# google-research/multinerf

Hardware: NVIDIA H100
Metric: train-step rays/sec @16384 rays x (64+64+32) samples (higher is better)
Workload: dtype bf16

## Files before the change

include/mnrf.h:

```cpp
#ifndef MNRF_H_
#define MNRF_H_

#include <stddef.h>
#include <stdint.h>

#ifdef __cplusplus
extern "C" {
#endif

typedef uint16_t mnrf_bf16;
typedef void* mnrf_stream;

#define MNRF_ABI_VERSION 1

int mnrf_abi_version(void);
const char* mnrf_last_error(void);
int mnrf_device_ok(void);
int mnrf_num_sms(void);

typedef struct {
  int32_t num_rays, num_prev, num_samples;
  int32_t use_dilation;
  float dilation, domain_lo, domain_hi;
  float anneal, resample_padding;
  int32_t jitter_mode;
  float max_jitter;
} mnrf_sample_desc;

int mnrf_sample_level(const mnrf_sample_desc* d, const float* sdist_prev, const float* w_prev,
                      const float* u_base, const float* jitter, const float* cw_in,
                      float* sdist_out, int32_t* idx_out, float* cw_out, float* tdil_out,
                      float* wdil_out, mnrf_stream stream);
int mnrf_sample_level_dyn(const mnrf_sample_desc* d, const float* sdist_prev, const float* w_prev,
                          const float* u_base, const float* jitter, const float* anneal_dev,
                          float* sdist_out, mnrf_stream stream);

enum { MNRF_RAYDIST_NONE = 0, MNRF_RAYDIST_RECIPROCAL, MNRF_RAYDIST_LOG, MNRF_RAYDIST_EXP,
       MNRF_RAYDIST_SQRT, MNRF_RAYDIST_SQUARE, MNRF_RAYDIST_PIECEWISE };
enum { MNRF_RAY_CONE = 0, MNRF_RAY_CYLINDER = 1 };

typedef struct {
  int32_t num_rays, num_samples;
  int32_t raydist_fn, ray_shape, warp_contract, disable_integration;
  int32_t basis_k, min_deg, max_deg;
  int32_t ld_feat, feat_cols;
} mnrf_encode_desc;

int mnrf_encode(const mnrf_encode_desc* d, const float* sdist, const float* origins,
                const float* directions, const float* radii, const float* near,
                const float* far, const float* basis, mnrf_bf16* feat_bf16, float* feat_f32,
                float* tdist_out, mnrf_stream stream);
int mnrf_encode_tangent(const mnrf_encode_desc* d, const float* sdist, const float* origins,
                        const float* directions, const float* radii, const float* near,
                        const float* far, const float* basis, mnrf_bf16* feat_bf16,
                        mnrf_bf16* tfeat_bf16, int32_t ld_tfeat, mnrf_stream stream);

int mnrf_viewdir_enc(int32_t num_rays, int32_t num_samples, int32_t deg, const float* viewdirs,
                     mnrf_bf16* out, int32_t ld, int32_t col0, int32_t col_end,
                     mnrf_stream stream);

enum { MNRF_GEMM_FWD = 0, MNRF_GEMM_DGRAD = 1, MNRF_GEMM_WGRAD = 2 };
enum { MNRF_ACT_NONE = 0, MNRF_ACT_RELU = 1, MNRF_ACT_SOFTPLUS = 2, MNRF_ACT_SILU = 3 };

typedef struct {
  int32_t mode, act;
  int64_t m;
  int32_t n, k;
  int64_t lda, ldb, ldc, ldmask;
  int64_t ldmaskbits;
  int64_t ldadd;
  int64_t mask_mod;
  int32_t impl;
} mnrf_gemm_desc;

int mnrf_gemm(const mnrf_gemm_desc* d, const mnrf_bf16* a, const mnrf_bf16* b, const float* bias,
              const float* rowv, const float* colv, const mnrf_bf16* mask, uint32_t* maskbits,
              float* colsum, const mnrf_bf16* addend, void* out, mnrf_stream stream);

int mnrf_gemm_act(const mnrf_gemm_desc* d, const mnrf_bf16* a, const mnrf_bf16* b, const float* bias,
                  const float* rowv, const float* colv, float* colsum, const mnrf_bf16* addend, mnrf_bf16* z,
                  int64_t ldz, void* out, mnrf_stream stream);

int mnrf_gemm_wgrad(const mnrf_gemm_desc* d, const mnrf_bf16* a, const mnrf_bf16* b, float* bsum,
                    const float* side_w, float* side_aw, float* out, mnrf_stream stream);

typedef struct {
  int32_t block_n;
  int32_t staged;
  int32_t mask_tma;
  int32_t smooth;
  int32_t side;
  int32_t splits;
  int32_t tiles;
  int32_t grid;
} mnrf_gemm_instance;
int mnrf_gemm_plan(const mnrf_gemm_desc* d, const mnrf_bf16* a, const mnrf_bf16* b, const float* bias,
                   const float* rowv, const float* colv, const mnrf_bf16* mask, const uint32_t* maskbits,
                   const float* colsum, const mnrf_bf16* addend, const mnrf_bf16* z, int64_t ldz, const void* out,
                   const float* bsum, const float* side_w, const float* side_aw, mnrf_gemm_instance* plan);

#define MNRF_CHAIN_MAX_LAYERS 8
enum { MNRF_CHAIN_FWD = 0, MNRF_CHAIN_BWD = 1 };

typedef struct {
  const mnrf_bf16* w;
  int64_t ldw;
  const float* bias;
  uint32_t* maskbits;
  int64_t ldmaskbits;
  float* colsum;
  mnrf_bf16* out;
  int64_t ldo;
  int32_t n_stream, stream_col0, stream_kb0;
  int32_t n_res, res_kb0;
  int32_t reserved;
} mnrf_chain_layer;

typedef struct {
  int32_t mode, num_layers;
  int32_t width;
  int32_t stream_cols;
  int64_t m;
  const mnrf_bf16* stream;
  int64_t ldstream;
  const float* head_w;
  const float* head_b;
  float* head_out;
  int32_t head_n;
  int32_t reserved;
  mnrf_chain_layer layer[MNRF_CHAIN_MAX_LAYERS];
} mnrf_chain_desc;

int mnrf_mlp_chain(const mnrf_chain_desc* d, mnrf_stream stream);
int mnrf_mlp_chain_max_layers(void);

int mnrf_head_fwd(int64_t m, int32_t k, int32_t n_out, const mnrf_bf16* x, int64_t ldx,
                  const mnrf_bf16* w, const float* b, float* raw, mnrf_stream stream);
int mnrf_head_bwd(int64_t m, int32_t k, int32_t n_out, const mnrf_bf16* x, int64_t ldx,
                  const mnrf_bf16* w, const float* draw, mnrf_bf16* dx, int64_t lddx,
                  int32_t relu_mask, float* dw, float* dw2, int32_t dw_split, float* db, float* dxsum,
                  int32_t dx_cols, mnrf_bf16* dx2, int64_t lddx2, mnrf_stream stream);
int mnrf_head_bwd_act(int64_t m, int32_t k, int32_t n_out, const mnrf_bf16* x, int64_t ldx,
                      const mnrf_bf16* w, const float* draw, mnrf_bf16* dx, int64_t lddx,
                      int32_t act, const mnrf_bf16* z, int64_t ldz, float* dw, float* dw2, int32_t dw_split,
                      float* db, float* dxsum, int32_t dx_cols, mnrf_bf16* dx2, int64_t lddx2, mnrf_stream stream);

int mnrf_colsum(int64_t m, int32_t n, const mnrf_bf16* x, int64_t ldx, float* out,
                mnrf_stream stream);

enum { MNRF_RGB_SIGMOID = 0, MNRF_RGB_SAFE_EXP = 1 };

typedef struct {
  int32_t num_rays, num_samples;
  int32_t raydist_fn, opaque_background;
  float density_bias, density_noise;
  int32_t rgb_act;
  float rgb_premult, rgb_bias, rgb_padding;
  float bg_const;
  int32_t rgb_mode;
  int32_t ld_density, ld_rgb;
} mnrf_composite_desc;

int mnrf_composite_fwd(const mnrf_composite_desc* d, const float* raw_density,
                       const float* raw_rgb, const float* density_noise, const float* sdist,
                       const float* directions, const float* near, const float* far,
                       const float* bg_rgb, const float* rgb_scale, const float* raw_diffuse,
                       const float* raw_tint, float* weights, float* rgb_out,
                       float* density_out, float* rgb_samples, float* acc, float* dist,
                       mnrf_stream stream);

enum { MNRF_LOSS_MSE = 0, MNRF_LOSS_CHARB = 1, MNRF_LOSS_RAWNERF = 2 };

typedef struct {
  mnrf_composite_desc c;
  int32_t loss_type;
  float charb_padding;
  float data_mult;
  float distortion_mult;
  float interlevel_mult;
  int32_t num_samples_fine;
  int32_t lossmult_channels;
} mnrf_loss_desc;

int mnrf_composite_bwd(const mnrf_loss_desc* d, const float* raw_density, const float* raw_rgb,
                       const float* density_noise, const float* sdist, const float* directions,
                       const float* near, const float* far, const float* bg_rgb,
                       const float* rgb_scale, const float* raw_diffuse, const float* raw_tint,
                       const float* extra_dw ,
                       const float* target_rgb,
                       const float* lossmult, const float* inv_denom ,
                       const float* sdist_fine, const float* weights_fine,
                       float* d_raw_density, float* d_raw_rgb, float* d_rgb_scale ,
                       float* d_raw_diffuse, float* d_raw_tint, float* stats, mnrf_stream stream);
int mnrf_composite_bwd_masked(const mnrf_loss_desc* d, const float* raw_density, const float* raw_rgb,
                              const float* density_noise, const float* sdist, const float* directions,
                              const float* near, const float* far, const float* bg_rgb,
                              const float* rgb_scale, const float* raw_diffuse, const float* raw_tint,
                              const float* extra_dw, const float* target_rgb,
                              const float* lossmult, const float* inv_denom,
                              const float* sdist_fine, const float* weights_fine, const float* data_mask,
                              float* d_raw_density, float* d_raw_rgb, float* d_rgb_scale,
                              float* d_raw_diffuse, float* d_raw_tint, float* stats, mnrf_stream stream);
int mnrf_composite_bwd_chunk(const mnrf_loss_desc* d, const float* raw_density, const float* raw_rgb,
                             const float* density_noise, const float* sdist, const float* directions,
                             const float* near, const float* far, const float* bg_rgb,
                             const float* rgb_scale, const float* raw_diffuse, const float* raw_tint,
                             const float* extra_dw, const float* target_rgb,
                             const float* lossmult, const float* inv_denom,
                             const float* sdist_fine, const float* weights_fine, const float* data_mask,
                             float* d_raw_density, float* d_raw_rgb, float* d_rgb_scale,
                             float* d_raw_diffuse, float* d_raw_tint, float* stats, int32_t batch_rays,
                             mnrf_stream stream);

typedef struct {
  int32_t num_rays;
  int32_t patch_size, inner_patch_size, filter_size;
  int32_t enable;
  float smoothed_thresh;
  float patch_thresh;
} mnrf_robust_desc;

int mnrf_robust_mask(const mnrf_robust_desc* d, const float* rgb, const float* target, const float* threshold,
                     float* mask, float* error_per_pixel, uint32_t* counts, float* stats, mnrf_stream stream);
int mnrf_robust_mask_chunk(const mnrf_robust_desc* d, const float* rgb, const float* target, const float* threshold,
                           float* mask, float* error_per_pixel, uint32_t* counts, float* stats, int32_t batch_rays,
                           mnrf_stream stream);
int mnrf_quantile(int32_t n, float q, const float* x, float* out, mnrf_stream stream);

typedef struct {
  int64_t M;
  int32_t num_samples;
  int32_t use_pred_normals, use_density_normals, use_reflections, use_ide, use_n_dot_v, use_roughness;
  int32_t deg_view, ide_n;
  float roughness_bias;
  int32_t ld, col0, col_end;
} mnrf_refdir_desc;

int mnrf_refdir_fwd(const mnrf_refdir_desc* d, const float* ide_mat, const int32_t* ide_ml,
                    const float* grad_pred, const float* raw_rough, const float* raw_grad_density,
                    const float* viewdirs, float* normals_pred, float* normals, float* roughness,
                    mnrf_bf16* slab, float orient_mult, float prednorm_mult, int32_t orient_on_pred,
                    float* extra_dw , mnrf_stream stream);
int mnrf_refdir_bwd(const mnrf_refdir_desc* d, const float* ide_mat, const int32_t* ide_ml,
                    const float* grad_pred, const float* raw_rough, const float* raw_grad_density,
                    const float* viewdirs, const float* weights, mnrf_bf16* d_slab,
                    int32_t ld_dslab, float orient_mult, float prednorm_mult, int32_t orient_on_pred,
                    const float* d_raw_density, const float* d_raw_diffuse, const float* d_raw_tint,
// ... 79 lines not shown
```

multinerf_b200/csrc/gemm_tc.cu:

```cuda
#include <cuda.h>

#include <stdlib.h>
#include <string.h>

#include <algorithm>

#include "tc_common.cuh"

namespace mnrf {

constexpr int BLOCK_M = 128;
constexpr int BLOCK_K = 64;
constexpr int A_STAGE_BYTES = BLOCK_M * BLOCK_K * 2;
constexpr int NUM_THREADS = 384;
constexpr int CS_MAX = 1024;
constexpr int gemm_stages(int bn) { return bn == 256 ? 4 : bn == 128 ? 6 : 8; }
constexpr int STAGING_BLOCK_BYTES = 64 * 128;
constexpr int staging_blocks(int mode, int bn, bool ts) {
  return !ts ? 0 : (mode == MNRF_GEMM_FWD && bn >= 128) ? 2 : 1;
}
constexpr int mask_words(int bn) { return bn >= 128 ? bn / 32 : 0; }
constexpr int MASK_BUFS = 2;
constexpr int dgrad_smem_bytes(int bn) { return 8 * bn * 4 + MASK_BUFS * BLOCK_M * mask_words(bn) * 4; }
constexpr int SIDE_SCRATCH = 96 * 8;
// ... 265 lines not shown
      const bool leader = (threadIdx.x & 127) == 0;
      const uint32_t c_row = smem_u32(smem_c) + c * (SB * STAGING_BLOCK_BYTES) + (r_in - 64 * c) * 128 + (cq << 1);
      int64_t rows[2];
      bool row_ok[2];
      float rv[2] = {0.f, 0.f};
      const uint32_t* mrow[2] = {nullptr, nullptr};
#pragma unroll
      for (int h = 0; h < 2; ++h) {
        rows[h] = (int64_t)m_blk * BLOCK_M + r_in + 8 * h;
        row_ok[h] = rows[h] < p.m;
        if (MODE == MNRF_GEMM_DGRAD && row_ok[h]) {
          if (p.rowv) rv[h] = p.rowv[rows[h]];
          if (p.maskbits && !mask_tma)
            mrow[h] = p.maskbits + (p.mask_mod > 0 ? rows[h] % p.mask_mod : rows[h]) * p.ldmaskbits;
        }
      }
      const uint32_t m_row = smem_u32(mask_s) + ((it % MASK_BUFS) * BLOCK_M + r_in) * (MW * 4);
      if (mask_tma) mbar_wait(&mask_full[it % MASK_BUFS], (it / MASK_BUFS) & 1, 5);
      uint32_t bits[2] = {0u, 0u};
      uint32_t mw[2] = {0u, 0u};
#pragma unroll
      for (int i = 0; i < BN / 8; ++i) {
        const int col = ncol0 + 8 * i + cq;
        if (TS && SB == 1 && (i & 7) == 0) {
          if (leader) tma_store_wait_read<0>();
          named_bar_sync(2 + c, 128);
        }
        if (MODE == MNRF_GEMM_DGRAD && p.maskbits && (i & 3) == 0) {
#pragma unroll
          for (int h = 0; h < 2; ++h)
            mw[h] = mask_tma ? ld_shared_u32(m_row + (8 * h * MW + (i >> 2)) * 4)
                             : row_ok[h] ? __ldg(mrow[h] + (col >> 5)) : 0u;
        }
        float v[2][2];
#pragma unroll
        for (int h = 0; h < 2; ++h) { v[h][0] = acc[4 * i + 2 * h]; v[h][1] = acc[4 * i + 2 * h + 1]; }
        if (MODE == MNRF_GEMM_FWD) {
          if (p.bias) {
            const float2 b = __ldg(reinterpret_cast<const float2*>(p.bias + col));
#pragma unroll
            for (int h = 0; h < 2; ++h) { v[h][0] += b.x; v[h][1] += b.y; }
          }
          if constexpr (SMOOTH) {
#pragma unroll
            for (int h = 0; h < 2; ++h) {
              if (p.mask && row_ok[h])
                *reinterpret_cast<uint32_t*>(const_cast<__nv_bfloat16*>(p.mask) + rows[h] * p.ldmask + col) =
                    pack_bf16(v[h][0], v[h][1]);
              v[h][0] = act_fwd(p.act, v[h][0]);
              v[h][1] = act_fwd(p.act, v[h][1]);
            }
          } else if (p.act == MNRF_ACT_RELU) {
#pragma unroll
            for (int h = 0; h < 2; ++h)
#pragma unroll
              for (int e = 0; e < 2; ++e) {
                v[h][e] = fmaxf(v[h][e], 0.f);
                bits[h] |= (v[h][e] > 0.f ? 1u : 0u) << ((8 * i + cq + e) & 31);
              }
          }
        } else {
          float2 cv = make_float2(0.f, 0.f);
          if (p.rowv) cv = __ldg(reinterpret_cast<const float2*>(p.colv + col));
#pragma unroll
          for (int h = 0; h < 2; ++h) {
            if (p.rowv) { v[h][0] += rv[h] * cv.x; v[h][1] += rv[h] * cv.y; }
            if constexpr (SMOOTH) {
              if (row_ok[h]) {
                const int64_t zr = p.mask_mod > 0 ? rows[h] % p.mask_mod : rows[h];
                const uint32_t zz = __ldg(reinterpret_cast<const unsigned int*>(p.mask + zr * p.ldmask + col));
                v[h][0] *= act_d1(p.act, bf16_lo(zz));
                v[h][1] *= act_d1(p.act, bf16_hi(zz));
              }
            } else if (p.maskbits) {
              if (!((mw[h] >> (col & 31)) & 1u)) v[h][0] = 0.f;
              if (!((mw[h] >> ((col + 1) & 31)) & 1u)) v[h][1] = 0.f;
            } else if (p.mask && row_ok[h]) {
              const uint32_t mm = __ldg(reinterpret_cast<const unsigned int*>(p.mask + rows[h] * p.ldmask + col));
              if (!(bf16_lo(mm) > 0.f)) v[h][0] = 0.f;
              if (!(bf16_hi(mm) > 0.f)) v[h][1] = 0.f;
            }
            if (p.addend && row_ok[h]) {
              const uint32_t aa = __ldg(reinterpret_cast<const unsigned int*>(p.addend + rows[h] * p.ldadd + col));
              v[h][0] += bf16_lo(aa);
              v[h][1] += bf16_hi(aa);
            }
          }
          if (do_cs) {
            const bool hi = (lane >> 2) & 1;
            const float s0 = v[0][0] + v[1][0], s1 = v[0][1] + v[1][1];
            float t = (hi ? s1 : s0) + __shfl_xor_sync(0xffffffffu, hi ? s0 : s1, 4);
            t += __shfl_xor_sync(0xffffffffu, t, 8);
            t += __shfl_xor_sync(0xffffffffu, t, 16);
            if (lane < 8) {
              const uint32_t a = cs_lane + 8 * i * 4;
              st_shared_u32(a, __float_as_uint(__uint_as_float(ld_shared_u32(a)) + t));
            }
          }
        }
#pragma unroll
        for (int h = 0; h < 2; ++h) {
          if (TS) {
            st_shared_u32(c_row + ((i >> 3) & (SB - 1)) * STAGING_BLOCK_BYTES + h * (8 * 128) +
                              (((i & 7) ^ ((lane >> 2) & 7)) << 4),
                          pack_bf16(v[h][0], v[h][1]));
          } else if (row_ok[h]) {
            *reinterpret_cast<uint32_t*>(reinterpret_cast<__nv_bfloat16*>(p.out) + rows[h] * p.ldc + col) =
                pack_bf16(v[h][0], v[h][1]);
          }
        }
        if (MODE == MNRF_GEMM_FWD && p.act == MNRF_ACT_RELU && p.maskbits && (i & 3) == 3) {
#pragma unroll
          for (int h = 0; h < 2; ++h) {
            bits[h] |= __shfl_xor_sync(0xffffffffu, bits[h], 1);
            bits[h] |= __shfl_xor_sync(0xffffffffu, bits[h], 2);
            if ((lane & 3) == ((i >> 2) & 3) && row_ok[h]) p.maskbits[rows[h] * p.ldmaskbits + (col >> 5)] = bits[h];
            bits[h] = 0u;
          }
        }
        if (TS && (i & 7) == 7) {
          fence_proxy_async();
          if (SB == 2 && leader) tma_store_wait_read<0>();
          named_bar_sync(2 + c, 128);
          if (leader) {
            tma_store_2d(&tmap_c, smem_c + (c * SB + ((i >> 3) & (SB - 1))) * STAGING_BLOCK_BYTES, ncol0 + 8 * (i & ~7),
                         (int)((int64_t)m_blk * BLOCK_M + 64 * c));
            tma_store_commit();
          }
        }
      }
      if (mask_tma) {
        __syncwarp();
        if (lane == 0) mbar_arrive(&mask_empty[it % MASK_BUFS]);
      }
      const int next = tile + (int)gridDim.x;
      if (do_cs && (next >= total_tiles || next % p.num_n_blocks != n_blk)) {
        named_bar_sync(1, 2 * 128);
        for (int j = threadIdx.x - 128; j < BN; j += 2 * 128) {
          float s = 0.f;
#pragma unroll
          for (int sw = 0; sw < 8; ++sw) {
            s += cs_s[sw * BN + j];
            cs_s[sw * BN + j] = 0.f;
          }
          atomicAdd(p.colsum + ncol0 + j, s);
        }
        named_bar_sync(1, 2 * 128);
      }
    }
    if (TS && (threadIdx.x & 127) == 0) tma_store_wait_all();
  }
}

template <int MODE, int BN, bool TS, bool SIDE, bool SMOOTH>
static int launch_gemm_tc(int grid, const CUtensorMap& ta, const CUtensorMap& tb, const CUtensorMap& tc,
                          const CUtensorMap& tm, const GemmParams& p, cudaStream_t stream) {
  static bool attr_set = false;
  constexpr int kSmem = smem_bytes(MODE, BN, TS, SIDE);
  static_assert(kSmem <= 232448, "shared memory budget");
  auto kern = gemm_tc_kernel<MODE, BN, TS, SIDE, SMOOTH>;
  if (!attr_set) {
    MNRF_CUDA(cudaFuncSetAttribute(kern, cudaFuncAttributeMaxDynamicSharedMemorySize, kSmem));
    attr_set = true;
  }
  cudaLaunchConfig_t cfg = {};
  cfg.gridDim = dim3(grid); cfg.blockDim = dim3(NUM_THREADS);
  cfg.dynamicSmemBytes = kSmem; cfg.stream = stream;
  cudaLaunchAttribute attr[1];
  attr[0].id = cudaLaunchAttributeProgrammaticStreamSerialization;
  attr[0].val.programmaticStreamSerializationAllowed = 1;
  cfg.attrs = attr; cfg.numAttrs = pdl_enabled() ? 1 : 0;
  MNRF_CUDA(cudaLaunchKernelEx(&cfg, kern, ta, tb, tc, tm, p));
  return 0;
}

int gemm_tc_smooth_launch(int mode, int block_n, int grid, const CUtensorMap& ta, const CUtensorMap& tb,
                          const CUtensorMap& tc, const GemmParams& p, cudaStream_t stream);

#ifndef MNRF_GEMM_TC_SMOOTH_UNIT
static int pick_block_n(int n) {
  const int cands[] = {256, 128, 64, 32, 16};
  for (int c : cands)
    if (n % c == 0) return c;
  return 0;
}

static int gemm_tc_plan(const mnrf_gemm_desc* d, const mnrf_bf16* a, const mnrf_bf16* b, const float* bias,
                        const float* colv, const mnrf_bf16* mask, const uint32_t* maskbits, const float* colsum,
                        const mnrf_bf16* addend, const void* out, const float* bsum, const float* side_w,
                        const float* side_aw, const mnrf_bf16* z, int64_t ldz, mnrf_gemm_instance* plan) {
  MNRF_CHECK(d->mode == MNRF_GEMM_WGRAD || d->k % BLOCK_K == 0,
             "mnrf_gemm(tc): reduction length %d must be a multiple of %d", d->k, BLOCK_K);
  MNRF_CHECK(d->lda % 8 == 0 && d->ldb % 8 == 0 && ((uintptr_t)a % 16) == 0 && ((uintptr_t)b % 16) == 0,
             "mnrf_gemm(tc): operands must be 16-byte aligned with ld %% 8 == 0");
  const int block_n = pick_block_n(d->n);
  MNRF_CHECK(block_n > 0, "mnrf_gemm(tc): N=%d must be a multiple of 16", d->n);
  if (d->mode == MNRF_GEMM_WGRAD)
    MNRF_CHECK(block_n >= 64, "mnrf_gemm(tc): WGRAD needs N %% 64 == 0 (MN-major 128-byte atoms), N=%d", d->n);
  if (addend) MNRF_CHECK(d->mode == MNRF_GEMM_DGRAD && d->ldadd % 2 == 0 && ((uintptr_t)addend % 4) == 0,
                         "mnrf_gemm(tc): addend is a DGRAD input with 4-byte aligned rows");
  if (colsum) MNRF_CHECK(d->mode == MNRF_GEMM_DGRAD && d->n <= CS_MAX,
                         "mnrf_gemm(tc): colsum is a DGRAD output of at most %d columns", CS_MAX);
  const bool side = bsum != nullptr || side_aw != nullptr;
  if (side) MNRF_CHECK(d->mode == MNRF_GEMM_WGRAD && (side_w == nullptr) == (side_aw == nullptr),
                       "mnrf_gemm(tc): side sums are WGRAD outputs; side_w and side_aw come together");
  if (maskbits) {
    MNRF_CHECK(d->mode != MNRF_GEMM_WGRAD, "mnrf_gemm(tc): maskbits make no sense for WGRAD");
    MNRF_CHECK(d->n % 32 == 0 && block_n % 32 == 0 && d->ldmaskbits * 32 >= d->n,
               "mnrf_gemm(tc): maskbits need N %% 32 == 0 and ldmaskbits >= N/32");
  }
  const bool smooth = d->mode != MNRF_GEMM_WGRAD && (d->act == MNRF_ACT_SOFTPLUS || d->act == MNRF_ACT_SILU);
  if (smooth) {
    MNRF_CHECK(!maskbits && !mask, "mnrf_gemm(tc): a smooth activation takes z, not a ReLU mask");
    MNRF_CHECK(d->mode == MNRF_GEMM_FWD || z, "mnrf_gemm(tc): the DGRAD of a smooth activation needs z");
    MNRF_CHECK(!z || (ldz % 2 == 0 && ((uintptr_t)z % 4) == 0), "mnrf_gemm(tc): z must be 4-byte aligned");
  }
  if (bias) MNRF_CHECK(((uintptr_t)bias % 8) == 0, "mnrf_gemm(tc): bias must be 8-byte aligned");
  if (colv) MNRF_CHECK(((uintptr_t)colv % 8) == 0, "mnrf_gemm(tc): colv must be 8-byte aligned");
  const int workers = mnrf_num_sms();
  const int num_m_blocks = (int)((d->m + BLOCK_M - 1) / BLOCK_M);
  const int num_n_blocks = d->n / block_n;
  const int num_k_blocks = (d->k + BLOCK_K - 1) / BLOCK_K;
  int num_splits = 1;
  if (d->mode == MNRF_GEMM_WGRAD) {
    const int out_tiles = num_m_blocks * num_n_blocks;
    const int max_splits = std::min(std::max(1, (2 * workers) / out_tiles), num_k_blocks);
    int splits = max_splits;
    for (int sp = 1; sp <= max_splits; ++sp) {
      const int items = out_tiles * sp;
      const int rounds = (items + workers - 1) / workers;
      if (items * 100 >= rounds * workers * 95) { splits = sp; break; }
    }
    num_splits = splits;
  }
  const int kblocks_per_split = (num_k_blocks + num_splits - 1) / num_splits;
  num_splits = (num_k_blocks + kblocks_per_split - 1) / kblocks_per_split;
  if (d->mode != MNRF_GEMM_WGRAD) {
    MNRF_CHECK(d->ldc % 2 == 0 && ((uintptr_t)out % 4) == 0, "mnrf_gemm(tc): bf16 output must be 4-byte aligned");
    if (mask) MNRF_CHECK(d->ldmask % 2 == 0 && ((uintptr_t)mask % 4) == 0, "mnrf_gemm(tc): mask must be 4-byte aligned");
  } else {
    MNRF_CHECK(d->ldc % 2 == 0 && ((uintptr_t)out % 8) == 0, "mnrf_gemm(tc): fp32 output must be 8-byte aligned");
  }
  const bool ts = d->mode != MNRF_GEMM_WGRAD && block_n >= 64 && ((uintptr_t)out % 16) == 0 && d->ldc % 8 == 0;
  MNRF_CHECK(!smooth || ts, "mnrf_gemm(tc): a smooth activation needs N %% 64 == 0 and a 16-byte aligned output "
             "with a row pitch that is a multiple of 8");
  const bool mask_tma = d->mode == MNRF_GEMM_DGRAD && maskbits && mask_words(block_n) > 0 && d->ldmaskbits % 4 == 0 &&
                        ((uintptr_t)maskbits % 16) == 0 && (d->mask_mod == 0 || d->mask_mod % BLOCK_M == 0);
  const int tiles = num_m_blocks * num_n_blocks * num_splits;
  plan->block_n = block_n;
  plan->staged = ts;
  plan->mask_tma = mask_tma;
  plan->smooth = smooth;
  plan->side = side;
  plan->splits = num_splits;
  plan->tiles = tiles;
  plan->grid = std::min(tiles, workers);
  return 0;
}

int gemm_tc_launch(const mnrf_gemm_desc* d, const mnrf_bf16* a, const mnrf_bf16* b, const float* bias,
                   const float* rowv, const float* colv, const mnrf_bf16* mask, uint32_t* maskbits,
                   float* colsum, const mnrf_bf16* addend, void* out, cudaStream_t stream, float* bsum,
                   const float* side_w, float* side_aw, mnrf_bf16* z, int64_t ldz) {
  mnrf_gemm_instance plan;
  if (int rc = gemm_tc_plan(d, a, b, bias, colv, mask, maskbits, colsum, addend, out, bsum, side_w, side_aw, z, ldz,
                            &plan))
    return rc;
  const int block_n = plan.block_n;
  const bool ts = plan.staged, side = plan.side, smooth = plan.smooth;
  GemmParams p{};
  p.mode = d->mode; p.act = d->act; p.m = d->m; p.n = d->n; p.k = d->k;
  p.num_m_blocks = (int)((d->m + BLOCK_M - 1) / BLOCK_M);
  p.num_n_blocks = d->n / block_n;
  p.num_k_blocks = (d->k + BLOCK_K - 1) / BLOCK_K;
  p.num_splits = plan.splits;
  p.kblocks_per_split = (p.num_k_blocks + p.num_splits - 1) / p.num_splits;
  p.ldc = d->ldc; p.ldmask = d->ldmask;
  p.bias = bias; p.rowv = rowv; p.colv = colv;
  p.mask = reinterpret_cast<const __nv_bfloat16*>(mask);
  p.out = out;
  p.maskbits = maskbits;
  p.ldmaskbits = d->ldmaskbits;
  p.mask_mod = d->mask_mod;
  p.addend = reinterpret_cast<const __nv_bfloat16*>(addend);
  p.ldadd = d->ldadd;
  p.colsum = colsum;
  p.bsum = bsum; p.side_w = side_w; p.side_aw = side_aw;
  if (smooth) {
    p.mask = reinterpret_cast<const __nv_bfloat16*>(z);
    p.ldmask = ldz;
  }
  p.mask_tma = plan.mask_tma;
  CUtensorMap ta, tb, tc;
  if (d->mode != MNRF_GEMM_WGRAD) {
    if (make_tmap(&ta, a, d->m, d->k, d->lda, BLOCK_K, BLOCK_M)) return 1;
    if (make_tmap(&tb, b, d->n, d->k, d->ldb, BLOCK_K, block_n)) return 1;
  } else {
    if (make_tmap(&ta, a, d->k, d->m, d->lda, 64, BLOCK_K)) return 1;
    if (make_tmap(&tb, b, d->k, d->n, d->ldb, 64, BLOCK_K)) return 1;
  }
  if (ts) {
    if (make_tmap(&tc, out, d->m, d->n, d->ldc, 64, 64)) return 1;
  } else {
    tc = tb;
  }
  CUtensorMap tm = tb;
  if (p.mask_tma &&
      make_tmap(&tm, maskbits, d->mask_mod > 0 ? d->mask_mod : d->m, d->n / 32, d->ldmaskbits,
                mask_words(block_n), BLOCK_M, CU_TENSOR_MAP_DATA_TYPE_UINT32, 4,
                CU_TENSOR_MAP_SWIZZLE_NONE))
    return 1;
  const int grid = plan.grid;
  if (grid == 0) return 0;
#define MNRF_LAUNCH_TC3(MODE_, BN_, TS_, SIDE_)                                                       \
  do {                                                                                                \
    if (int rc = launch_gemm_tc<MODE_, BN_, TS_, SIDE_, false>(grid, ta, tb, tc, tm, p, stream)) return rc; \
  } while (0)
#define MNRF_LAUNCH_TC2(MODE_, BN_)                                                                   \
  do {                                                                                                \
    if (side) MNRF_LAUNCH_TC3(MODE_, BN_, false, MODE_ == MNRF_GEMM_WGRAD && BN_ >= 64);              \
    else if (ts) MNRF_LAUNCH_TC3(MODE_, BN_, MODE_ != MNRF_GEMM_WGRAD && BN_ >= 64, false);           \
    else MNRF_LAUNCH_TC3(MODE_, BN_, false, false);                                                   \
  } while (0)
#define MNRF_LAUNCH_TC(MODE_)                                                                         \
  do {                                                                                                \
    switch (block_n) {                                                                                \
      case 256: MNRF_LAUNCH_TC2(MODE_, 256); break;                                                   \
      case 128: MNRF_LAUNCH_TC2(MODE_, 128); break;                                                   \
      case 64: MNRF_LAUNCH_TC2(MODE_, 64); break;                                                     \
      case 32: if (MODE_ != MNRF_GEMM_WGRAD) MNRF_LAUNCH_TC2(MODE_, 32); break;                       \
      default: if (MODE_ != MNRF_GEMM_WGRAD) MNRF_LAUNCH_TC2(MODE_, 16); break;                       \
    }                                                                                                 \
  } while (0)
  if (smooth) {
    if (int rc = gemm_tc_smooth_launch(d->mode, block_n, grid, ta, tb, tc, p, stream)) return rc;
  } else if (d->mode == MNRF_GEMM_FWD) MNRF_LAUNCH_TC(MNRF_GEMM_FWD);
  else if (d->mode == MNRF_GEMM_DGRAD) MNRF_LAUNCH_TC(MNRF_GEMM_DGRAD);
  else MNRF_LAUNCH_TC(MNRF_GEMM_WGRAD);
  MNRF_LAUNCH_CHECK();
  return 0;
}
#endif

}

#ifndef MNRF_GEMM_TC_SMOOTH_UNIT
extern "C" int mnrf_gemm_plan(const mnrf_gemm_desc* d, const mnrf_bf16* a, const mnrf_bf16* b, const float* bias,
                              const float* rowv, const float* colv, const mnrf_bf16* mask, const uint32_t* maskbits,
                              const float* colsum, const mnrf_bf16* addend, const mnrf_bf16* z, int64_t ldz,
                              const void* out, const float* bsum, const float* side_w, const float* side_aw,
                              mnrf_gemm_instance* plan) {
  MNRF_CHECK(d && plan, "mnrf_gemm_plan: null pointer");
  MNRF_CHECK((rowv == nullptr) == (colv == nullptr), "mnrf_gemm: rowv and colv come together");
  MNRF_CHECK(!mask || d->mask_mod == 0, "mnrf_gemm: mask_mod applies to maskbits and z, not to a bf16 mask");
  return mnrf::gemm_tc_plan(d, a, b, bias, colv, mask, maskbits, colsum, addend, out, bsum, side_w, side_aw, z, ldz,
                            plan);
}
#endif
```

multinerf_b200/lib.py:

```python
import ctypes as C
import os

import torch

_HERE = os.path.dirname(os.path.abspath(__file__))
LIB_PATH = os.environ.get('MNRF_LIB') or os.path.join(_HERE, 'libmnrf_b200.so')


class MnrfError(RuntimeError):
  pass


class SampleDesc(C.Structure):
  _fields_ = [('num_rays', C.c_int32), ('num_prev', C.c_int32), ('num_samples', C.c_int32),
              ('use_dilation', C.c_int32), ('dilation', C.c_float), ('domain_lo', C.c_float),
              ('domain_hi', C.c_float), ('anneal', C.c_float), ('resample_padding', C.c_float),
              ('jitter_mode', C.c_int32), ('max_jitter', C.c_float)]


class EncodeDesc(C.Structure):
  _fields_ = [('num_rays', C.c_int32), ('num_samples', C.c_int32), ('raydist_fn', C.c_int32),
              ('ray_shape', C.c_int32), ('warp_contract', C.c_int32),
              ('disable_integration', C.c_int32), ('basis_k', C.c_int32), ('min_deg', C.c_int32),
              ('max_deg', C.c_int32), ('ld_feat', C.c_int32), ('feat_cols', C.c_int32)]


class GemmDesc(C.Structure):
  _fields_ = [('mode', C.c_int32), ('act', C.c_int32), ('m', C.c_int64), ('n', C.c_int32),
              ('k', C.c_int32), ('lda', C.c_int64), ('ldb', C.c_int64), ('ldc', C.c_int64),
              ('ldmask', C.c_int64), ('ldmaskbits', C.c_int64), ('ldadd', C.c_int64),
              ('mask_mod', C.c_int64),
              ('impl', C.c_int32)]


class GemmInstance(C.Structure):
  _fields_ = [('block_n', C.c_int32), ('staged', C.c_int32), ('mask_tma', C.c_int32), ('smooth', C.c_int32),
              ('side', C.c_int32), ('splits', C.c_int32), ('tiles', C.c_int32), ('grid', C.c_int32)]


class CompositeDesc(C.Structure):
  _fields_ = [('num_rays', C.c_int32), ('num_samples', C.c_int32), ('raydist_fn', C.c_int32),
              ('opaque_background', C.c_int32), ('density_bias', C.c_float),
              ('density_noise', C.c_float), ('rgb_act', C.c_int32), ('rgb_premult', C.c_float),
              ('rgb_bias', C.c_float), ('rgb_padding', C.c_float), ('bg_const', C.c_float),
              ('rgb_mode', C.c_int32), ('ld_density', C.c_int32), ('ld_rgb', C.c_int32)]


class LossDesc(C.Structure):
  _fields_ = [('c', CompositeDesc), ('loss_type', C.c_int32), ('charb_padding', C.c_float),
              ('data_mult', C.c_float), ('distortion_mult', C.c_float),
              ('interlevel_mult', C.c_float), ('num_samples_fine', C.c_int32),
              ('lossmult_channels', C.c_int32)]


class RobustDesc(C.Structure):
  _fields_ = [('num_rays', C.c_int32), ('patch_size', C.c_int32), ('inner_patch_size', C.c_int32),
              ('filter_size', C.c_int32), ('enable', C.c_int32), ('smoothed_thresh', C.c_float),
              ('patch_thresh', C.c_float)]


class RefdirDesc(C.Structure):
  _fields_ = [('M', C.c_int64), ('num_samples', C.c_int32), ('use_pred_normals', C.c_int32),
              ('use_density_normals', C.c_int32), ('use_reflections', C.c_int32), ('use_ide', C.c_int32),
              ('use_n_dot_v', C.c_int32), ('use_roughness', C.c_int32), ('deg_view', C.c_int32),
              ('ide_n', C.c_int32), ('roughness_bias', C.c_float), ('ld', C.c_int32), ('col0', C.c_int32),
              ('col_end', C.c_int32)]


class CameraDesc(C.Structure):
  _fields_ = [('num_rays', C.c_int32), ('num_cameras', C.c_int32), ('camtype', C.c_int32),
              ('has_distortion', C.c_int32), ('k1', C.c_float), ('k2', C.c_float), ('k3', C.c_float),
              ('k4', C.c_float), ('p1', C.c_float), ('p2', C.c_float), ('undistort_eps', C.c_float),
              ('undistort_iters', C.c_int32), ('has_ndc', C.c_int32), ('ndc_p02', C.c_float),
              ('ndc_p12', C.c_float), ('ndc_near', C.c_float)]


class SphericalDesc(C.Structure):
  _fields_ = [('height', C.c_int32), ('width', C.c_int32), ('camtoworld', C.c_double * 12)]


class PackItem(C.Structure):
  _fields_ = [('master', C.c_void_p), ('w_nk', C.c_void_p), ('w_kn', C.c_void_p), ('in_pad', C.c_int32),
              ('out', C.c_int32), ('tile0', C.c_int32), ('reserved', C.c_int32)]


CHAIN_MAX_LAYERS = 8
CHAIN_FWD, CHAIN_BWD = 0, 1


class ChainLayer(C.Structure):
  _fields_ = [('w', C.c_void_p), ('ldw', C.c_int64), ('bias', C.c_void_p), ('maskbits', C.c_void_p),
              ('ldmaskbits', C.c_int64), ('colsum', C.c_void_p), ('out', C.c_void_p), ('ldo', C.c_int64),
              ('n_stream', C.c_int32), ('stream_col0', C.c_int32), ('stream_kb0', C.c_int32),
              ('n_res', C.c_int32), ('res_kb0', C.c_int32), ('reserved', C.c_int32)]


class ChainDesc(C.Structure):
  _fields_ = [('mode', C.c_int32), ('num_layers', C.c_int32), ('width', C.c_int32), ('stream_cols', C.c_int32),
              ('m', C.c_int64), ('stream', C.c_void_p), ('ldstream', C.c_int64), ('head_w', C.c_void_p),
              ('head_b', C.c_void_p), ('head_out', C.c_void_p), ('head_n', C.c_int32), ('reserved', C.c_int32),
              ('layer', ChainLayer * CHAIN_MAX_LAYERS)]


class AdamDesc(C.Structure):
  _fields_ = [('n', C.c_int64), ('grad_max_val', C.c_float), ('grad_max_norm', C.c_float),
              ('lr', C.c_float), ('beta1', C.c_float), ('beta2', C.c_float), ('eps', C.c_float),
              ('step', C.c_int32), ('grad_scale', C.c_float)]


RAYDIST = {None: 0, 'none': 0, 'reciprocal': 1, 'log': 2, 'exp': 3, 'sqrt': 4, 'square': 5,
           'piecewise': 6}
RAY_SHAPE = {'cone': 0, 'cylinder': 1}
RGB_ACT = {'sigmoid': 0, 'safe_exp': 1}
LOSS_TYPE = {'mse': 0, 'charb': 1, 'rawnerf': 2}
GEMM_FWD, GEMM_DGRAD, GEMM_WGRAD = 0, 1, 2
ACT_NONE, ACT_RELU, ACT_SOFTPLUS, ACT_SILU = 0, 1, 2, 3
SMOOTH_ACTS = (ACT_SOFTPLUS, ACT_SILU)

_P = C.c_void_p
_SIGNATURES = {
    'mnrf_abi_version': (C.c_int, []),
    'mnrf_last_error': (C.c_char_p, []),
    'mnrf_device_ok': (C.c_int, []),
    'mnrf_num_sms': (C.c_int, []),
    'mnrf_sample_level': (C.c_int, [C.POINTER(SampleDesc)] + [_P] * 11),
    'mnrf_sample_level_dyn': (C.c_int, [C.POINTER(SampleDesc)] + [_P] * 7),
    'mnrf_encode': (C.c_int, [C.POINTER(EncodeDesc)] + [_P] * 11),
    'mnrf_viewdir_enc': (C.c_int, [C.c_int32, C.c_int32, C.c_int32, _P, _P, C.c_int32, C.c_int32,
                                   C.c_int32, _P]),
    'mnrf_gemm': (C.c_int, [C.POINTER(GemmDesc)] + [_P] * 11),
    'mnrf_gemm_act': (C.c_int, [C.POINTER(GemmDesc)] + [_P] * 8 + [C.c_int64, _P, _P]),
    'mnrf_gemm_wgrad': (C.c_int, [C.POINTER(GemmDesc)] + [_P] * 7),
    'mnrf_gemm_plan': (C.c_int, [C.POINTER(GemmDesc)] + [_P] * 10 + [C.c_int64] + [_P] * 4 +
                       [C.POINTER(GemmInstance)]),
    'mnrf_mlp_chain': (C.c_int, [C.POINTER(ChainDesc), _P]),
    'mnrf_mlp_chain_max_layers': (C.c_int, []),
    'mnrf_head_fwd': (C.c_int, [C.c_int64, C.c_int32, C.c_int32, _P, C.c_int64, _P, _P, _P, _P]),
    'mnrf_head_bwd': (C.c_int, [C.c_int64, C.c_int32, C.c_int32, _P, C.c_int64, _P, _P, _P,
                                C.c_int64, C.c_int32, _P, _P, C.c_int32, _P, _P, C.c_int32, _P, C.c_int64, _P]),
    'mnrf_head_bwd_act': (C.c_int, [C.c_int64, C.c_int32, C.c_int32, _P, C.c_int64, _P, _P, _P, C.c_int64,
                                    C.c_int32, _P, C.c_int64, _P, _P, C.c_int32, _P, _P, C.c_int32, _P, C.c_int64,
                                    _P]),
    'mnrf_colsum': (C.c_int, [C.c_int64, C.c_int32, _P, C.c_int64, _P, _P]),
    'mnrf_composite_fwd': (C.c_int, [C.POINTER(CompositeDesc)] + [_P] * 18),
    'mnrf_composite_bwd': (C.c_int, [C.POINTER(LossDesc)] + [_P] * 24),
    'mnrf_composite_bwd_masked': (C.c_int, [C.POINTER(LossDesc)] + [_P] * 25),
    'mnrf_composite_bwd_chunk': (C.c_int, [C.POINTER(LossDesc)] + [_P] * 24 + [C.c_int32, _P]),
    'mnrf_robust_mask': (C.c_int, [C.POINTER(RobustDesc)] + [_P] * 8),
    'mnrf_robust_mask_chunk': (C.c_int, [C.POINTER(RobustDesc)] + [_P] * 7 + [C.c_int32, _P]),
    'mnrf_quantile': (C.c_int, [C.c_int32, C.c_float, _P, _P, _P]),
    'mnrf_encode_tangent': (C.c_int, [C.POINTER(EncodeDesc)] + [_P] * 9 + [C.c_int32, _P]),
    'mnrf_refdir_fwd': (C.c_int, [C.POINTER(RefdirDesc)] + [_P] * 10 + [C.c_float, C.c_float, C.c_int32, _P, _P]),
    'mnrf_refdir_bwd': (C.c_int, [C.POINTER(RefdirDesc)] + [_P] * 8 + [C.c_int32, C.c_float, C.c_float, C.c_int32] +
                        [_P] * 8),
    'mnrf_normals_fwd': (C.c_int, [C.c_int64, C.c_int32] + [_P] * 5 + [C.c_float, C.c_float, C.c_int32, _P, _P]),
    'mnrf_normals_bwd': (C.c_int, [C.c_int64, C.c_int32] + [_P] * 4 + [C.c_float, C.c_float, C.c_int32] + [_P] * 2 +
                         [C.c_int64] + [_P] * 3 +
                         [C.c_int64, _P, _P]),
    'mnrf_outer_mask': (C.c_int,[C.c_int64, C.c_int32, C.c_int64, _P, _P, _P, C.c_int64, _P, C.c_int64, _P]),
    'mnrf_act_tangent_bwd': (C.c_int, [C.c_int64, C.c_int32, C.c_int32] + [_P, C.c_int64] * 5 + [C.c_int32, _P]),
    'mnrf_pixels_to_rays': (C.c_int, [C.POINTER(CameraDesc)] + [_P] * 11),
    'mnrf_spherical_rays': (C.c_int, [C.POINTER(SphericalDesc)] + [_P] * 6),
    'mnrf_clip_adam': (C.c_int, [C.POINTER(AdamDesc)] + [_P] * 6),
    'mnrf_clip_adam_dyn': (C.c_int, [C.POINTER(AdamDesc)] + [_P] * 7),
    'mnrf_pack_weights': (C.c_int, [C.c_int32, C.c_int32, _P, _P, _P, _P]),
    'mnrf_pack_weights_batched': (C.c_int, [C.c_int32, _P, C.c_int32, _P]),
}
EXPORTED = tuple(_SIGNATURES)

_lib = None


def load(build_if_missing=False):
  global _lib
  if _lib is not None:
    return _lib
  if not os.path.exists(LIB_PATH):
    if build_if_missing:
      from . import build as _build
      _build.build()
    else:
      raise MnrfError(f'{LIB_PATH} is missing: run `python -m multinerf_b200.build` '
                      '(there is no CPU fallback)')
  lib = C.CDLL(LIB_PATH)
  for name, (res, args) in _SIGNATURES.items():
    fn = getattr(lib, name)
    fn.restype = res
    fn.argtypes = args
  if lib.mnrf_abi_version() != 1:
    raise MnrfError('ABI version mismatch')
# ... 29 lines not shown
```

Before: 246,300.

## Add ping-pong warpgroup GEMM kernel for FWD and DGRAD tiles

Adds a persistent ping-pong GEMM kernel in which two consumer warpgroups alternate whole 128-column sub-tiles. One warpgroup runs its epilogue (bias, ReLU, masking, TMA store) while the other issues WGMMA, with an mbarrier turn token ordering the two. The planner picks this path for non-WGRAD GEMMs with a staged output, N divisible by 128, no smooth activation and no colsum. It trades fewer pipeline stages and a narrower N per warpgroup for hiding the epilogue behind the MMAs, and adds ordering complexity between the warpgroups.

```diff
diff --git a/include/mnrf.h b/include/mnrf.h
--- a/include/mnrf.h
+++ b/include/mnrf.h
@@ -93,6 +93,7 @@
   int32_t splits;
   int32_t tiles;
   int32_t grid;
+  int32_t pingpong;
 } mnrf_gemm_instance;
 int mnrf_gemm_plan(const mnrf_gemm_desc* d, const mnrf_bf16* a, const mnrf_bf16* b, const float* bias,
                    const float* rowv, const float* colv, const mnrf_bf16* mask, const uint32_t* maskbits,
diff --git a/multinerf_b200/csrc/gemm_tc.cu b/multinerf_b200/csrc/gemm_tc.cu
--- a/multinerf_b200/csrc/gemm_tc.cu
+++ b/multinerf_b200/csrc/gemm_tc.cu
@@ -441,6 +441,273 @@
   }
 }
 
+constexpr int PP_BN = 128;
+constexpr int PP_STAGES = 5;
+constexpr int PP_SB = 2;
+constexpr int PP_MASK_BUFS = 4;
+constexpr int pp_smem_bytes(int mode) {
+  return PP_STAGES * (A_STAGE_BYTES + PP_BN * BLOCK_K * 2) + 2 * PP_SB * STAGING_BLOCK_BYTES +
+         (mode == MNRF_GEMM_DGRAD ? PP_MASK_BUFS * BLOCK_M * mask_words(PP_BN) * 4 : 0) + 256  +
+         1024 ;
+}
+
+template <int MODE, int BN>
+__global__ void __launch_bounds__(NUM_THREADS, 1)
+gemm_tc_pingpong_kernel(const __grid_constant__ CUtensorMap tmap_a, const __grid_constant__ CUtensorMap tmap_b,
+                        const __grid_constant__ CUtensorMap tmap_c, const __grid_constant__ CUtensorMap tmap_m,
+                        const GemmParams p) {
+  constexpr int STAGES = PP_STAGES;
+  constexpr int B_STAGE = PP_BN * BLOCK_K * 2;
+  constexpr int SUB = BN / PP_BN;
+  constexpr int MW = mask_words(PP_BN);
+  constexpr int SB = PP_SB;
+  constexpr bool kDgrad = (MODE == MNRF_GEMM_DGRAD);
+  static_assert(MODE != MNRF_GEMM_WGRAD && (BN == 128 || BN == 256), "FWD / DGRAD tiles of 128 or 256 columns");
+  extern __shared__ uint8_t smem_dyn[];
+  uint8_t* smem = reinterpret_cast<uint8_t*>((reinterpret_cast<uintptr_t>(smem_dyn) + 1023) & ~uintptr_t(1023));
+  uint8_t* smem_a = smem;
+  uint8_t* smem_b = smem + STAGES * A_STAGE_BYTES;
+  uint8_t* smem_c = smem_b + STAGES * B_STAGE;
+  uint32_t* mask_s = reinterpret_cast<uint32_t*>(smem_c + 2 * SB * STAGING_BLOCK_BYTES);
+  uint64_t* full_bar = reinterpret_cast<uint64_t*>(mask_s + (kDgrad ? PP_MASK_BUFS * BLOCK_M * MW : 0));
+  uint64_t* empty_bar = full_bar + STAGES;
+  uint64_t* mask_full = empty_bar + STAGES;
+  uint64_t* mask_empty = mask_full + PP_MASK_BUFS;
+  uint64_t* mma_turn = mask_empty + PP_MASK_BUFS;
+
+  const int warp = threadIdx.x >> 5;
+  const int lane = threadIdx.x & 31;
+  const int wg = threadIdx.x >> 7;
+  const int total_tiles = p.num_m_blocks * p.num_n_blocks;
+  const int nk = p.num_k_blocks;
+  const bool mask_tma = kDgrad && p.mask_tma;
+
+  if (threadIdx.x == 0) {
+    prefetch_tmap(&tmap_a);
+    prefetch_tmap(&tmap_b);
+    prefetch_tmap(&tmap_c);
+    if (mask_tma) prefetch_tmap(&tmap_m);
+    for (int i = 0; i < STAGES; ++i) {
+      mbar_init(&full_bar[i], 1);
+      mbar_init(&empty_bar[i], 4);
+    }
+    for (int i = 0; i < PP_MASK_BUFS; ++i) {
+      mbar_init(&mask_full[i], 1);
+      mbar_init(&mask_empty[i], 4);
+    }
+    for (int i = 0; i < 2; ++i) mbar_init(&mma_turn[i], 4);
+    fence_barrier_init();
+  }
+  __syncthreads();
+  pdl_launch_dependents();
+  pdl_wait();
+
+  if (wg == 0) {
+    setmaxnreg_dec<40>();
+    if (threadIdx.x == 0) {
+      uint32_t stage = 0, phase = 0;
+      int it = 0;
+      for (int tile = blockIdx.x; tile < total_tiles; tile += gridDim.x) {
+        const int n_blk = tile % p.num_n_blocks;
+        const int m_blk = tile / p.num_n_blocks;
+        for (int s = 0; s < SUB; ++s, ++it) {
+          const int ncol0 = n_blk * BN + s * PP_BN;
+          if (mask_tma) {
+            const int mb = it % PP_MASK_BUFS;
+            mbar_wait(&mask_empty[mb], ((it / PP_MASK_BUFS) & 1) ^ 1, 4);
+            mbar_expect_tx(&mask_full[mb], BLOCK_M * MW * 4);
+            const int64_t r0 = (int64_t)m_blk * BLOCK_M;
+            tma_load_2d(mask_s + mb * (BLOCK_M * MW), &tmap_m, &mask_full[mb], ncol0 / 32,
+                        (int)(p.mask_mod > 0 ? r0 % p.mask_mod : r0));
+          }
+          for (int kb = 0; kb < nk; ++kb) {
+            mbar_wait(&empty_bar[stage], phase ^ 1, 1);
+            mbar_expect_tx(&full_bar[stage], A_STAGE_BYTES + B_STAGE);
+            tma_load_2d(smem_a + stage * A_STAGE_BYTES, &tmap_a, &full_bar[stage], kb * BLOCK_K, m_blk * BLOCK_M);
+            tma_load_2d(smem_b + stage * B_STAGE, &tmap_b, &full_bar[stage], kb * BLOCK_K, ncol0);
+            if (++stage == STAGES) { stage = 0; phase ^= 1; }
+          }
+        }
+      }
+    }
+  } else {
+    setmaxnreg_inc<232>();
+    const int c = wg - 1;
+    const int w = warp & 3;
+    const int cq = 2 * (lane & 3);
+    const bool leader = (threadIdx.x & 127) == 0;
+    const uint32_t c_row = smem_u32(smem_c) + c * (SB * STAGING_BLOCK_BYTES) + (16 * w + (lane >> 2)) * 128 + (cq << 1);
+    float acc[2][64];
+    for (int it = c; ; it += 2) {
+      const int tile = blockIdx.x + (it / SUB) * (int)gridDim.x;
+      if (tile >= total_tiles) break;
+      const int s = it % SUB;
+      const int n_blk = tile % p.num_n_blocks;
+      const int m_blk = tile / p.num_n_blocks;
+      const int ncol0 = n_blk * BN + s * PP_BN;
+      const uint32_t slot = (uint32_t)it * (uint32_t)nk;
+      uint32_t stage = slot % STAGES, phase = (slot / STAGES) & 1;
+      if (it > 0) mbar_wait(&mma_turn[c], ((it - 1) >> 1) & 1, 7);
+      int prev = -1;
+      fence_acc(acc[0]);
+      fence_acc(acc[1]);
+      for (int kb = 0; kb < nk; ++kb) {
+        mbar_wait(&full_bar[stage], phase, 3);
+        const uint32_t sa = smem_u32(smem_a + stage * A_STAGE_BYTES);
+        const uint32_t sb = smem_u32(smem_b + stage * B_STAGE);
+        wgmma_fence();
+#pragma unroll
+        for (int k = 0; k < BLOCK_K / WGMMA_K; ++k) {
+          const uint64_t bdesc = make_smem_desc(sb + k * (WGMMA_K * 2), 0, 1024);
+#pragma unroll
+          for (int g = 0; g < 2; ++g)
+            Wgmma<PP_BN, 0, 0>::mma(acc[g], make_smem_desc(sa + g * (64 * 128) + k * (WGMMA_K * 2), 0, 1024), bdesc,
+                                    (kb > 0 || k > 0) ? 1u : 0u);
+        }
+        wgmma_commit();
+        wgmma_wait<1>();
+        if (prev >= 0 && lane == 0) mbar_arrive(&empty_bar[prev]);
+        prev = (int)stage;
+        if (++stage == STAGES) { stage = 0; phase ^= 1; }
+      }
+      if (blockIdx.x + ((it + 1) / SUB) * (int)gridDim.x < total_tiles) {
+        __syncwarp();
+        if (lane == 0) mbar_arrive(&mma_turn[c ^ 1]);
+      }
+      wgmma_wait<0>();
+      fence_acc(acc[0]);
+      fence_acc(acc[1]);
+      if (prev >= 0 && lane == 0) mbar_arrive(&empty_bar[prev]);
+
+      const uint32_t m_base = smem_u32(mask_s) + (it % PP_MASK_BUFS) * (BLOCK_M * MW * 4);
+      if (mask_tma) mbar_wait(&mask_full[it % PP_MASK_BUFS], (it / PP_MASK_BUFS) & 1, 5);
+#pragma unroll 1
+      for (int g = 0; g < 2; ++g) {
+        const int r_in = 64 * g + 16 * w + (lane >> 2);
+        int64_t rows[2];
+        bool row_ok[2];
+        float rv[2] = {0.f, 0.f};
+        const uint32_t* mrow[2] = {nullptr, nullptr};
+#pragma unroll
+        for (int h = 0; h < 2; ++h) {
+          rows[h] = (int64_t)m_blk * BLOCK_M + r_in + 8 * h;
+          row_ok[h] = rows[h] < p.m;
+          if (kDgrad && row_ok[h]) {
+            if (p.rowv) rv[h] = p.rowv[rows[h]];
+            if (p.maskbits && !mask_tma)
+              mrow[h] = p.maskbits + (p.mask_mod > 0 ? rows[h] % p.mask_mod : rows[h]) * p.ldmaskbits;
+          }
+        }
+        const uint32_t m_row = m_base + r_in * (MW * 4);
+        uint32_t bits[2] = {0u, 0u};
+        uint32_t mw[2] = {0u, 0u};
+#pragma unroll
+        for (int i = 0; i < PP_BN / 8; ++i) {
+          const int col = ncol0 + 8 * i + cq;
+          if (kDgrad && p.maskbits && (i & 3) == 0) {
+#pragma unroll
+            for (int h = 0; h < 2; ++h)
+              mw[h] = mask_tma ? ld_shared_u32(m_row + (8 * h * MW + (i >> 2)) * 4)
+                               : row_ok[h] ? __ldg(mrow[h] + (col >> 5)) : 0u;
+          }
+          float v[2][2];
+#pragma unroll
+          for (int h = 0; h < 2; ++h) { v[h][0] = acc[0][4 * i + 2 * h]; v[h][1] = acc[0][4 * i + 2 * h + 1]; }
+          if (!kDgrad) {
+            if (p.bias) {
+              const float2 b = __ldg(reinterpret_cast<const float2*>(p.bias + col));
+#pragma unroll
+              for (int h = 0; h < 2; ++h) { v[h][0] += b.x; v[h][1] += b.y; }
+            }
+            if (p.act == MNRF_ACT_RELU) {
+#pragma unroll
+              for (int h = 0; h < 2; ++h)
+#pragma unroll
+                for (int e = 0; e < 2; ++e) {
+                  v[h][e] = fmaxf(v[h][e], 0.f);
+                  bits[h] |= (v[h][e] > 0.f ? 1u : 0u) << ((8 * i + cq + e) & 31);
+                }
+            }
+          } else {
+            float2 cv = make_float2(0.f, 0.f);
+            if (p.rowv) cv = __ldg(reinterpret_cast<const float2*>(p.colv + col));
+#pragma unroll
+            for (int h = 0; h < 2; ++h) {
+              if (p.rowv) { v[h][0] += rv[h] * cv.x; v[h][1] += rv[h] * cv.y; }
+              if (p.maskbits) {
+                if (!((mw[h] >> (col & 31)) & 1u)) v[h][0] = 0.f;
+                if (!((mw[h] >> ((col + 1) & 31)) & 1u)) v[h][1] = 0.f;
+              } else if (p.mask && row_ok[h]) {
+                const uint32_t mm = __ldg(reinterpret_cast<const unsigned int*>(p.mask + rows[h] * p.ldmask + col));
+                if (!(bf16_lo(mm) > 0.f)) v[h][0] = 0.f;
+                if (!(bf16_hi(mm) > 0.f)) v[h][1] = 0.f;
+              }
+              if (p.addend && row_ok[h]) {
+                const uint32_t aa = __ldg(reinterpret_cast<const unsigned int*>(p.addend + rows[h] * p.ldadd + col));
+                v[h][0] += bf16_lo(aa);
+                v[h][1] += bf16_hi(aa);
+              }
+            }
+          }
+#pragma unroll
+          for (int h = 0; h < 2; ++h)
+            st_shared_u32(c_row + ((i >> 3) & (SB - 1)) * STAGING_BLOCK_BYTES + h * (8 * 128) +
+                              (((i & 7) ^ ((lane >> 2) & 7)) << 4),
+                          pack_bf16(v[h][0], v[h][1]));
+          if (!kDgrad && p.act == MNRF_ACT_RELU && p.maskbits && (i & 3) == 3) {
+#pragma unroll
+            for (int h = 0; h < 2; ++h) {
+              bits[h] |= __shfl_xor_sync(0xffffffffu, bits[h], 1);
+              bits[h] |= __shfl_xor_sync(0xffffffffu, bits[h], 2);
+              if ((lane & 3) == ((i >> 2) & 3) && row_ok[h]) p.maskbits[rows[h] * p.ldmaskbits + (col >> 5)] = bits[h];
+              bits[h] = 0u;
+            }
+          }
+          if ((i & 7) == 7) {
+            fence_proxy_async();
+            if (leader) tma_store_wait_read<0>();
+            named_bar_sync(2 + c, 128);
+            if (leader) {
+              tma_store_2d(&tmap_c, smem_c + (c * SB + ((i >> 3) & (SB - 1))) * STAGING_BLOCK_BYTES,
+                           ncol0 + 8 * (i & ~7), (int)((int64_t)m_blk * BLOCK_M + 64 * g));
+              tma_store_commit();
+            }
+          }
+        }
+#pragma unroll
+        for (int e = 0; e < 64; ++e) acc[0][e] = acc[1][e];
+      }
+      if (mask_tma) {
+        __syncwarp();
+        if (lane == 0) mbar_arrive(&mask_empty[it % PP_MASK_BUFS]);
+      }
+    }
+    if ((threadIdx.x & 127) == 0) tma_store_wait_all();
+  }
+}
+
+template <int MODE, int BN>
+static int launch_gemm_tc_pingpong(int grid, const CUtensorMap& ta, const CUtensorMap& tb, const CUtensorMap& tc,
+                                   const CUtensorMap& tm, const GemmParams& p, cudaStream_t stream) {
+  static bool attr_set = false;
+  constexpr int kSmem = pp_smem_bytes(MODE);
+  static_assert(kSmem <= 232448, "shared memory budget");
+  auto kern = gemm_tc_pingpong_kernel<MODE, BN>;
+  if (!attr_set) {
+    MNRF_CUDA(cudaFuncSetAttribute(kern, cudaFuncAttributeMaxDynamicSharedMemorySize, kSmem));
+    attr_set = true;
+  }
+  cudaLaunchConfig_t cfg = {};
+  cfg.gridDim = dim3(grid); cfg.blockDim = dim3(NUM_THREADS);
+  cfg.dynamicSmemBytes = kSmem; cfg.stream = stream;
+  cudaLaunchAttribute attr[1];
+  attr[0].id = cudaLaunchAttributeProgrammaticStreamSerialization;
+  attr[0].val.programmaticStreamSerializationAllowed = 1;
+  cfg.attrs = attr; cfg.numAttrs = pdl_enabled() ? 1 : 0;
+  MNRF_CUDA(cudaLaunchKernelEx(&cfg, kern, ta, tb, tc, tm, p));
+  return 0;
+}
+
 template <int MODE, int BN, bool TS, bool SIDE, bool SMOOTH>
 static int launch_gemm_tc(int grid, const CUtensorMap& ta, const CUtensorMap& tb, const CUtensorMap& tc,
                           const CUtensorMap& tm, const GemmParams& p, cudaStream_t stream) {
@@ -535,6 +802,7 @@
              "with a row pitch that is a multiple of 8");
   const bool mask_tma = d->mode == MNRF_GEMM_DGRAD && maskbits && mask_words(block_n) > 0 && d->ldmaskbits % 4 == 0 &&
                         ((uintptr_t)maskbits % 16) == 0 && (d->mask_mod == 0 || d->mask_mod % BLOCK_M == 0);
+  const bool pingpong = d->mode != MNRF_GEMM_WGRAD && ts && d->n % PP_BN == 0 && !smooth && !colsum;
   const int tiles = num_m_blocks * num_n_blocks * num_splits;
   plan->block_n = block_n;
   plan->staged = ts;
@@ -544,6 +812,7 @@
   plan->splits = num_splits;
   plan->tiles = tiles;
   plan->grid = std::min(tiles, workers);
+  plan->pingpong = pingpong;
   return 0;
 }
 
@@ -583,7 +852,7 @@
   CUtensorMap ta, tb, tc;
   if (d->mode != MNRF_GEMM_WGRAD) {
     if (make_tmap(&ta, a, d->m, d->k, d->lda, BLOCK_K, BLOCK_M)) return 1;
-    if (make_tmap(&tb, b, d->n, d->k, d->ldb, BLOCK_K, block_n)) return 1;
+    if (make_tmap(&tb, b, d->n, d->k, d->ldb, BLOCK_K, plan.pingpong ? PP_BN : block_n)) return 1;
   } else {
     if (make_tmap(&ta, a, d->k, d->m, d->lda, 64, BLOCK_K)) return 1;
     if (make_tmap(&tb, b, d->k, d->n, d->ldb, 64, BLOCK_K)) return 1;
@@ -596,7 +865,7 @@
   CUtensorMap tm = tb;
   if (p.mask_tma &&
       make_tmap(&tm, maskbits, d->mask_mod > 0 ? d->mask_mod : d->m, d->n / 32, d->ldmaskbits,
-                mask_words(block_n), BLOCK_M, CU_TENSOR_MAP_DATA_TYPE_UINT32, 4,
+                mask_words(plan.pingpong ? PP_BN : block_n), BLOCK_M, CU_TENSOR_MAP_DATA_TYPE_UINT32, 4,
                 CU_TENSOR_MAP_SWIZZLE_NONE))
     return 1;
   const int grid = plan.grid;
@@ -621,7 +890,17 @@
       default: if (MODE_ != MNRF_GEMM_WGRAD) MNRF_LAUNCH_TC2(MODE_, 16); break;                       \
     }                                                                                                 \
   } while (0)
-  if (smooth) {
+  if (plan.pingpong) {
+    const bool fwd = d->mode == MNRF_GEMM_FWD;
+    int rc;
+    if (block_n == 256)
+      rc = fwd ? launch_gemm_tc_pingpong<MNRF_GEMM_FWD, 256>(grid, ta, tb, tc, tm, p, stream)
+               : launch_gemm_tc_pingpong<MNRF_GEMM_DGRAD, 256>(grid, ta, tb, tc, tm, p, stream);
+    else
+      rc = fwd ? launch_gemm_tc_pingpong<MNRF_GEMM_FWD, 128>(grid, ta, tb, tc, tm, p, stream)
+               : launch_gemm_tc_pingpong<MNRF_GEMM_DGRAD, 128>(grid, ta, tb, tc, tm, p, stream);
+    if (rc) return rc;
+  } else if (smooth) {
     if (int rc = gemm_tc_smooth_launch(d->mode, block_n, grid, ta, tb, tc, p, stream)) return rc;
   } else if (d->mode == MNRF_GEMM_FWD) MNRF_LAUNCH_TC(MNRF_GEMM_FWD);
   else if (d->mode == MNRF_GEMM_DGRAD) MNRF_LAUNCH_TC(MNRF_GEMM_DGRAD);
diff --git a/multinerf_b200/lib.py b/multinerf_b200/lib.py
--- a/multinerf_b200/lib.py
+++ b/multinerf_b200/lib.py
@@ -35,7 +35,8 @@
 
 class GemmInstance(C.Structure):
   _fields_ = [('block_n', C.c_int32), ('staged', C.c_int32), ('mask_tma', C.c_int32), ('smooth', C.c_int32),
-              ('side', C.c_int32), ('splits', C.c_int32), ('tiles', C.c_int32), ('grid', C.c_int32)]
+              ('side', C.c_int32), ('splits', C.c_int32), ('tiles', C.c_int32), ('grid', C.c_int32),
+              ('pingpong', C.c_int32)]
 
 
 class CompositeDesc(C.Structure):
```

Result: faster. 254,200 (median of 6 runs) (+3.2%).
